# leggedrobotics/qed-splatter

Hardware: AMD Instinct MI355X
Metric: train iters/sec @ 1080p, 500k Gaussians (fwd + loss + bwd + Adam; camera-steps/s over all GPUs) (higher is better)
Workload: dtype f32

## Files before the change

### qed_splatter_amd/_lib.py

```python
from __future__ import annotations

import ctypes as C
import os
import types
from pathlib import Path

_LIB = None
LIB_PATH = Path(__file__).resolve().parent / "lib" / "libqed_splat.so"

_P = C.c_void_p
_I = C.c_int32
_L = C.c_int64
_F = C.c_float
_U = C.c_uint32
_D = C.c_double
_Q = C.c_uint64
SIGNATURES = {
    "qed_version": (C.c_int, []),
    "qed_last_error": (C.c_char_p, []),
    "qed_camera_setup": (C.c_int, [_I, _P, _P, _P, _P, _P]),
    "qed_project_fwd": (C.c_int, [_I, _I, _P, _P, _P, _P, _P, _I, _P, _I, _I, _P, _P, _I, _I, _I, _I, _F, _F, _F,
                                  _F, _U, _P, _P, _P, _P, _P, _P, _P, _P, _P, _P, _P, _P, _P, _P]),
    "qed_project_bwd": (C.c_int, [_I, _I, _P, _P, _P, _P, _P, _I, _P, _I, _I, _P, _P, _I, _I, _F, _U, _P, _P, _P,
                                  _P, _P, _P, _P, _I, _P, _I, _P, _P, _P]),
# ... 121 lines not shown
F_LOG_SCALES = 2
F_LOGIT_OPAC = 4
F_DEPTH_CHANNEL = 8
F_SIGMOID_COLORS = 16
F_TIGHT_TILES = 32
F_CAMERA_C2W = 128
F_SH_GRAD_COMPACT = 64
SPLAT_FLOATS = 12
VSPLAT_FLOATS = 16
SH_JAC_FLOATS = 10
STATUS_WORDS = 4
TILE = 16
CL_TILE_WAVES, CL_QUADRANT_WAVES, CL_HALF_AND_HALF, CL_NO_CULL, CL_ORDER_READY = 1, 2, 3, 4, 8
NN_NATURAL_ORDER, NN_AUTO_CELL = 1, 2
KNN_SKIP_FIRST = 4
BIN_AUTO, BIN_TWO_STAGE, BIN_TILE_SORT, BIN_BUCKET = 0, 1, 2, 3


def bin_mode() -> int:
    return {"two": BIN_TWO_STAGE, "til": BIN_TILE_SORT, "buc": BIN_BUCKET}.get(os.environ.get("QED_BIN_MODE", "")[:3],
                                                                            BIN_AUTO)


def composite_launch_flags() -> int:
    f = {"t": CL_TILE_WAVES, "q": CL_QUADRANT_WAVES, "h": CL_HALF_AND_HALF}.get(
        os.environ.get("QED_COMPOSITE_WAVES", "")[:1], 0)
    if os.environ.get("QED_COMPOSITE_NOCULL", "")[:1] == "1":
        f |= CL_NO_CULL
    return f


class QedSplatError(RuntimeError):
    pass


ABI_VERSION = 4


def load():
    global _LIB
    if _LIB is not None:
        return _LIB
    import torch
    path = Path(os.environ.get("QED_SPLAT_LIB", LIB_PATH))
    if not path.exists():
        raise QedSplatError(
# ... 102 lines not shown
```

### qed_splatter_amd/binning.py

```python
from __future__ import annotations

import time
import warnings
import weakref
from typing import Dict

import torch

from . import _lib as L


def pinned_slot():
    import ctypes
    host = torch.zeros(4, dtype=torch.int32).pin_memory()
    dptr = ctypes.c_void_p()
    L.check(L.load().qed_host_device_pointer(host.data_ptr(), ctypes.addressof(dptr)), "qed_host_device_pointer")
    return host.numpy(), dptr.value, host


class _Workspace:

    HEADROOM = 2.0
    POLL_TIMEOUT_S = 20.0

# ... 126 lines not shown
                  size=None, tile_masks=None, capture_slot=None):
    lib = L.load()
    dev = means2d.device
    ws = _workspace(dev)
    n_tiles = tile_w * tile_h
    key = (tuple(size) if size is not None else (tile_w, tile_h), N, C)
    n_isect = ws.n_isect
    offsets = torch.empty(C * n_tiles + 1, dtype=torch.int32, device=dev)
    capturing = torch.cuda.is_current_stream_capturing()
    if capturing:
        if not ws.may_capture(key):
            raise L.QedSplatError("run one eager call of this shape (image size, number of Gaussians, cameras) before "
                                  "capturing: it calibrates the intersection capacity")
        sync = False
    else:
        ws.poll_pending()
        if not ws.may_skip_readback(key):
            sync = True
    if ws.capacity == 0:
        ws.capacity = max(1 << 16, 8 * C * N)
    mode = L.bin_mode()
    if mode == L.BIN_AUTO and ws.m_seen.get(key, 0) > 0:
        mode = L.BIN_BUCKET if int(1.25 * ws.m_seen[key]) <= 1024 * C * n_tiles else L.BIN_TWO_STAGE
    host = host_ptr = None
    if not sync and not capturing:
        host, host_ptr = ws.host_slot()
    elif capturing and capture_slot is not None:
        host, host_ptr = capture_slot
    for _attempt in range(2):
        cap = ws.capacity
        flatten_ids = torch.empty(cap, dtype=torch.int32, device=dev)
        isect_ids = torch.empty(cap, dtype=torch.int64, device=dev) if sync else None
        scratch = torch.empty(int(lib.qed_bin_workspace_bytes(C * N, cap)), dtype=torch.uint8, device=dev)
        L.check(lib.qed_bin_tiles(N, C, L.ptr(means2d), L.ptr(radii), L.ptr(depths), L.ptr(tiles_per_gauss), L.ptr(splats),
                                  L.ptr(tile_masks), L.ptr(block_sums), tile_w, tile_h, cap, mode, L.ptr(flatten_ids), L.ptr(offsets),
                                  L.ptr(n_isect), L.ptr(isect_ids), L.ptr(scratch), scratch.numel(), L.ptr(ws.status),
                                  host_ptr, L.current_stream()), "qed_bin_tiles")
        if capturing:
            return None, flatten_ids, offsets, None
        if not sync:
            ws.arm_pending(host, key)
            return None, flatten_ids, offsets, None
        M, overflow, watchdog = ws.read_words()
        if watchdog:
            ws.watchdog_fired("the radix-sort look-back watchdog fired: the list of this frame is mis-sorted")
        if overflow == 0:
# ... 7 lines not shown
```

### qed_splatter_amd/csrc/isect.hip

```cpp
#include "qed_common.h"

namespace qed {

constexpr int kScanPer = 32;
__global__ void __launch_bounds__(1024)
isect_scan_kernel(const int* __restrict__ block_sums, int n_blocks, int* __restrict__ block_offsets,
                  int* __restrict__ n_isect, long long capacity, int* __restrict__ status) {
    __shared__ long long wave_tot[16];
    __shared__ long long carry_s;
    const int tid = threadIdx.x, lane = tid & 63, wid = tid >> 6;
    if (tid == 0) carry_s = 0;
    __syncthreads();
    for (int base = 0; base < n_blocks; base += 1024 * kScanPer) {
        const int i0 = base + tid * kScanPer;
        int v[kScanPer];
        const bool vec = (((uintptr_t)block_sums | (uintptr_t)block_offsets) & 15) == 0;
        if (vec && i0 + kScanPer <= n_blocks) {
#pragma unroll
            for (int j = 0; j < kScanPer / 4; ++j) {
                const int4 q = reinterpret_cast<const int4*>(block_sums + i0)[j];
                v[4 * j] = q.x; v[4 * j + 1] = q.y; v[4 * j + 2] = q.z; v[4 * j + 3] = q.w;
            }
        } else {
#pragma unroll
// ... 256 lines not shown
    int v = 0;
    if (i < n_slots) {
        if (order == nullptr) {
            v = tiles_per_gauss[i];
        } else if (slot_bits >= 32) {
            v = tiles_per_gauss[order[i]];
        } else {
            const unsigned o = (unsigned)order[i], marker = (1u << (32 - slot_bits)) - 1u;
            const unsigned c = o >> slot_bits;
            v = c == marker ? tiles_per_gauss[o & ((1u << slot_bits) - 1u)] : (int)c;
        }
    }
    __shared__ int wsum[4];
    v = wave_sum_i(v);
    if ((threadIdx.x & 63) == 0) wsum[threadIdx.x >> 6] = v;
    __syncthreads();
    if (threadIdx.x == 0) block_sums[blockIdx.x] = wsum[0] + wsum[1] + wsum[2] + wsum[3];
}


constexpr int kTileSortKpt = 8;
constexpr int kTileSortItems = 256 * kTileSortKpt;

__device__ __forceinline__ int wave_digit_rank(bool valid, unsigned d, int* cnt, int lane) {
    unsigned long long peers = __ballot(valid);
#pragma unroll
    for (int b = 0; b < 8; ++b) {
        const bool bit = (d >> b) & 1u;
        const unsigned long long bal = __ballot(bit);
        peers &= bit ? bal : ~bal;
    }
    int r = 0;
    if (valid) {
        r = cnt[d] + __popcll(peers & ((1ull << lane) - 1ull));
        if ((peers >> lane) == 1ull) cnt[d] = r + 1;
    }
    return r;
}


constexpr int kTileWaveKpt = 8;
constexpr int kTileWaveItems = 64 * kTileWaveKpt;
constexpr int kTileBuckets = 512;
constexpr int kTileBucketMax = 12;

__device__ __forceinline__ void wave_lds_fence() {
    __builtin_amdgcn_fence(__ATOMIC_ACQ_REL, "wavefront");
    __builtin_amdgcn_wave_barrier();
}

__device__ __forceinline__ void tile_sort_wave(int start, int n, int lane, uint2* __restrict__ kv, int* __restrict__ cnt,
                                               const int* __restrict__ vals_in, const float* __restrict__ depths,
                                               int* __restrict__ vals_out) {
    if (n == 1) {
        if (lane == 0) vals_out[start] = vals_in[start];
        return;
    }
    const int rows = (n + 63) >> 6;
    unsigned key[kTileWaveKpt];
    int val[kTileWaveKpt], rank[kTileWaveKpt];
#pragma unroll
    for (int k = 0; k < kTileWaveKpt; ++k) {
        if (k >= rows) break;
        const int li = k * 64 + lane;
        val[k] = vals_in[start + (li < n ? li : n - 1)];
    }
    unsigned kmin = 0xFFFFFFFFu, kmax = 0u;
#pragma unroll
    for (int k = 0; k < kTileWaveKpt; ++k) {
        if (k >= rows) break;
        key[k] = __float_as_uint(depths[val[k]]);
        kmin = min(kmin, key[k]);
        kmax = max(kmax, key[k]);
    }
#pragma unroll
    for (int o = 32; o > 0; o >>= 1) {
        kmin = min(kmin, (unsigned)__shfl_xor((int)kmin, o, 64));
        kmax = max(kmax, (unsigned)__shfl_xor((int)kmax, o, 64));
    }
    if (kmin == kmax) {
#pragma unroll
        for (int k = 0; k < kTileWaveKpt; ++k) {
            if (k >= rows) break;
            if (k * 64 + lane < n) vals_out[start + k * 64 + lane] = val[k];
        }
        return;
    }
    const float scale = 511.99f / (float)(kmax - kmin);
    unsigned bkt[kTileWaveKpt];
    *reinterpret_cast<int4*>(&cnt[8 * lane]) = make_int4(0, 0, 0, 0);
    *reinterpret_cast<int4*>(&cnt[8 * lane + 4]) = make_int4(0, 0, 0, 0);
    wave_lds_fence();
#pragma unroll
    for (int k = 0; k < kTileWaveKpt; ++k) {
        if (k >= rows) break;
        bkt[k] = min((unsigned)((float)(key[k] - kmin) * scale), (unsigned)(kTileBuckets - 1));
        rank[k] = k * 64 + lane < n ? atomicAdd(&cnt[bkt[k]], 1) : 0;
    }
    wave_lds_fence();
    int largest;
    {
        const int4 c0 = *reinterpret_cast<const int4*>(&cnt[8 * lane]);
        const int4 c1 = *reinterpret_cast<const int4*>(&cnt[8 * lane + 4]);
        largest = max(max(max(c0.x, c0.y), max(c0.z, c0.w)), max(max(c1.x, c1.y), max(c1.z, c1.w)));
        const int tot = c0.x + c0.y + c0.z + c0.w + c1.x + c1.y + c1.z + c1.w;
        int x = tot;
#pragma unroll
        for (int o = 1; o < 64; o <<= 1) {
            const int y = __shfl_up(x, o, 64);
            if (lane >= o) x += y;
        }
#pragma unroll
        for (int o = 32; o > 0; o >>= 1) largest = max(largest, __shfl_xor(largest, o, 64));
        int b = x - tot;
        int4 e0, e1;
        e0.x = b; b += c0.x; e0.y = b; b += c0.y; e0.z = b; b += c0.z; e0.w = b; b += c0.w;
        e1.x = b; b += c1.x; e1.y = b; b += c1.y; e1.z = b; b += c1.z; e1.w = b;
        *reinterpret_cast<int4*>(&cnt[8 * lane]) = e0;
        *reinterpret_cast<int4*>(&cnt[8 * lane + 4]) = e1;
    }
    wave_lds_fence();
    if (largest <= kTileBucketMax) {
#pragma unroll
        for (int k = 0; k < kTileWaveKpt; ++k) {
            if (k >= rows) break;
            if (k * 64 + lane < n) kv[cnt[bkt[k]] + rank[k]] = make_uint2(key[k], (unsigned)val[k]);
        }
        wave_lds_fence();
#pragma unroll
        for (int k = 0; k < kTileWaveKpt; ++k) {
            if (k >= rows) break;
            const int li = k * 64 + lane;
            if (li < n) {
                const int b0 = cnt[bkt[k]];
                const int b1 = bkt[k] + 1 < kTileBuckets ? cnt[bkt[k] + 1] : n;
                int before = 0;
                for (int j = b0; j < b1; ++j) {
                    const unsigned other = kv[j].x;
                    before += (other < key[k]) | ((other == key[k]) & ((int)kv[j].y < val[k]));
                }
                vals_out[start + b0 + before] = val[k];
            }
        }
        return;
    }
    unsigned* skeys = reinterpret_cast<unsigned*>(kv);
    int* svals = reinterpret_cast<int*>(kv) + kTileWaveItems;
    for (int pass = 0; pass < 4; ++pass) {
        const int shift = 8 * pass;
        *reinterpret_cast<int4*>(&cnt[4 * lane]) = make_int4(0, 0, 0, 0);
        wave_lds_fence();
#pragma unroll
        for (int k = 0; k < kTileWaveKpt; ++k) {
            if (k >= rows) break;
            rank[k] = wave_digit_rank(k * 64 + lane < n, (key[k] >> shift) & 255u, cnt, lane);
        }
        wave_lds_fence();
        const int4 c = *reinterpret_cast<const int4*>(&cnt[4 * lane]);
// ... 16 lines not shown
            const int li = k * 64 + lane;
            if (li < n) {
                const int pos = skip ? li : cnt[(key[k] >> shift) & 255u] + rank[k];
                if (last) vals_out[start + pos] = val[k];
                else { skeys[pos] = key[k]; svals[pos] = val[k]; }
            }
        }
        if (last) break;
        wave_lds_fence();
#pragma unroll
        for (int k = 0; k < kTileWaveKpt; ++k) {
            if (k >= rows) break;
            const int li = k * 64 + lane;
            if (li < n) { key[k] = skeys[li]; val[k] = svals[li]; }
        }
        wave_lds_fence();
    }
}

__device__ __forceinline__ void tile_sort_long_run(int start, int n, const int* __restrict__ vals_in,
                                                   const float* __restrict__ depths, int* __restrict__ vals_out,
                                                   unsigned* __restrict__ gk0, unsigned* __restrict__ gk1,
                                                   int* __restrict__ gv0, int* __restrict__ gv1, unsigned* s_keys,
                                                   int* s_vals, int (*s_cnt)[256], int* s_base, int* s_wsum, int* s_skip) {
    const int tid = threadIdx.x, lane = tid & 63, wid = tid >> 6;
    auto digit_scan = [&](int tot) {
        int x = tot;
#pragma unroll
        for (int o = 1; o < 64; o <<= 1) {
            const int y = __shfl_up(x, o, 64);
            if (lane >= o) x += y;
        }
        if (lane == 63) s_wsum[wid] = x;
        __syncthreads();
        int wb = 0;
        for (int w = 0; w < wid; ++w) wb += s_wsum[w];
        return wb + x - tot;
    };
    if (n <= kTileSortItems) {
        unsigned key[kTileSortKpt];
        int val[kTileSortKpt], rank[kTileSortKpt];
        const int Q = ((n + 255) >> 8) << 6;
        const int rows = Q >> 6;
        const int wbase = wid * Q;
        auto mine = [&](int k) { return wbase + 64 * k + lane < n; };
        if (tid < 4) s_skip[tid] = 0;
#pragma unroll
// ... 3 lines not shown
            val[k] = vals_in[start + (li < n ? li : n - 1)];
        }
#pragma unroll
        for (int k = 0; k < kTileSortKpt; ++k) {
            if (k >= rows) break;
            key[k] = __float_as_uint(depths[val[k]]);
        }
        for (int pass = 0; pass < 4; ++pass) {
            const int shift = 8 * pass;
#pragma unroll
            for (int w = 0; w < 4; ++w) s_cnt[w][tid] = 0;
            __syncthreads();
#pragma unroll
            for (int k = 0; k < kTileSortKpt; ++k) {
                if (k >= rows) break;
                rank[k] = wave_digit_rank(mine(k), (key[k] >> shift) & 255u, s_cnt[wid], lane);
            }
            __syncthreads();
            {
                int c[4], tot = 0;
#pragma unroll
                for (int w = 0; w < 4; ++w) c[w] = s_cnt[w][tid];
#pragma unroll
                for (int w = 0; w < 4; ++w) { s_cnt[w][tid] = tot; tot += c[w]; }
                if (tot == n) s_skip[pass] = 1;
                s_base[tid] = digit_scan(tot);
            }
            __syncthreads();
            const bool skip = s_skip[pass] != 0;
            const bool last = pass == 3;
            if (skip && !last) continue;
#pragma unroll
            for (int k = 0; k < kTileSortKpt; ++k) {
                if (k >= rows) break;
                if (mine(k)) {
                    const unsigned d = (key[k] >> shift) & 255u;
                    const int pos = skip ? wbase + k * 64 + lane : s_base[d] + s_cnt[wid][d] + rank[k];
                    if (last) vals_out[start + pos] = val[k];
                    else { s_keys[pos] = key[k]; s_vals[pos] = val[k]; }
                }
            }
            if (last) break;
            __syncthreads();
#pragma unroll
            for (int k = 0; k < kTileSortKpt; ++k) {
                if (k >= rows) break;
                if (mine(k)) { key[k] = s_keys[wbase + k * 64 + lane]; val[k] = s_vals[wbase + k * 64 + lane]; }
// ... 10 lines not shown
        s_base[tid] = 0;
        __syncthreads();
        for (int i = tid; i < n; i += 256) {
            const unsigned kk = ksrc ? ksrc[start + i] : __float_as_uint(depths[vsrc[start + i]]);
            atomicAdd(&s_base[(kk >> shift) & 255u], 1);
        }
        __syncthreads();
        const int tot = s_base[tid];
        const int base = digit_scan(tot);
        __syncthreads();
        s_base[tid] = base;
        __syncthreads();
        for (int row = 0; row < n; row += 256) {
            const int i = row + tid;
            const bool valid = i < n;
            const int vv = valid ? vsrc[start + i] : 0;
            const unsigned kk = valid ? (ksrc ? ksrc[start + i] : __float_as_uint(depths[vv])) : 0u;
            const unsigned d = (kk >> shift) & 255u;
#pragma unroll
            for (int w = 0; w < 4; ++w) s_cnt[w][tid] = 0;
            __syncthreads();
            const int r = wave_digit_rank(valid, d, s_cnt[wid], lane);
            __syncthreads();
            {
                int c[4], t2 = 0;
#pragma unroll
                for (int w = 0; w < 4; ++w) c[w] = s_cnt[w][tid];
                const int cur = s_base[tid];
#pragma unroll
                for (int w = 0; w < 4; ++w) { s_cnt[w][tid] = cur + t2; t2 += c[w]; }
                __syncthreads();
                s_base[tid] = cur + t2;
            }
            __syncthreads();
            if (valid) {
                const int pos = s_cnt[wid][d] + r;
                vdst[start + pos] = vv;
                if (pass < 3) kdst[start + pos] = kk;
            }
            __syncthreads();
        }
        __threadfence_block();
        __syncthreads();
        ksrc = kdst;
        vsrc = vdst;
    }
}

__global__ void __launch_bounds__(256)
tile_depth_sort_kernel(const int* __restrict__ offsets, const int* __restrict__ vals_in, const float* __restrict__ depths,
                       int* __restrict__ vals_out, unsigned* __restrict__ gk0, unsigned* __restrict__ gk1,
                       int* __restrict__ gv0, int* __restrict__ gv1, int n_tiles_total) {
    __shared__ __attribute__((aligned(16))) uint2 s_kv[4][kTileWaveItems];
    __shared__ __attribute__((aligned(16))) int s_cnt[4][kTileBuckets];
    __shared__ int s_wsum[4], s_skip[4];
    const int lane = threadIdx.x & 63, wid = threadIdx.x >> 6;
    const int tile = blockIdx.x * 4 + wid;
    int start = 0, n = 0;
    if (tile < n_tiles_total) { start = offsets[tile]; n = offsets[tile + 1] - start; }
    if (n >= 1 && n <= kTileWaveItems) tile_sort_wave(start, n, lane, s_kv[wid], s_cnt[wid], vals_in, depths, vals_out);
    if (!__syncthreads_or(n > kTileWaveItems)) return;
    static_assert(sizeof(s_kv) >= kTileSortItems * 8 && sizeof(s_cnt) >= (4 * 256 + 256) * 4, "LDS aliasing");
    unsigned* keys = reinterpret_cast<unsigned*>(&s_kv[0][0]);
    int* vals = reinterpret_cast<int*>(keys + kTileSortItems);
    int (*cnt)[256] = reinterpret_cast<int (*)[256]>(&s_cnt[0][0]);
    int* base = &s_cnt[0][0] + 4 * 256;
    for (int j = 0; j < 4; ++j) {
        const int t = blockIdx.x * 4 + j;
        if (t >= n_tiles_total) break;
        const int s0 = offsets[t], m = offsets[t + 1] - s0;
        if (m <= kTileWaveItems) continue;
        __syncthreads();
        tile_sort_long_run(s0, m, vals_in, depths, vals_out, gk0, gk1, gv0, gv1, keys, vals, cnt, base, s_wsum, s_skip);
    }
}

constexpr int kPartThreads = 1024;
constexpr int kPartWaves = kPartThreads / 64;
constexpr int kPartRows = 16;
constexpr int kPartStage = 32768;

__global__ void __launch_bounds__(kPartThreads)
bucket_partition_kernel(const unsigned* __restrict__ keys, const int* __restrict__ vals, const int* __restrict__ n_dev,
                        const int* __restrict__ bucket_tot, int low_bits, int tile_bits, int n_tiles,
                        int n_tiles_total, int* __restrict__ vals_out, unsigned* __restrict__ keys_out,
                        int* __restrict__ offsets, const int* __restrict__ status, int* __restrict__ host_words) {
    __shared__ int s_cnt[kPartWaves][256];
    __shared__ int s_base[256];
    __shared__ int s_wsum[4][2];
    __shared__ int s_stage[kPartStage];
    const int tid = threadIdx.x, lane = tid & 63, wid = tid >> 6;
    const int b = blockIdx.x;
    const int n = n_dev[0];
    if (b == 0 && tid == 0) {
        offsets[n_tiles_total] = n;
        if (host_words != nullptr) {
            *reinterpret_cast<int4*>(host_words) = make_int4(n, status[0], status[1], 0);
            __threadfence_system();
        }
    }
    const unsigned dmask = (1u << low_bits) - 1u;
    int before = 0, size = 0;
    if (tid < 256) {
        const int t = bucket_tot[tid];
        before = tid < b ? t : 0;
        if (tid == b) size = t;
    }
    before = wave_sum_i(before); size = wave_sum_i(size);
    if (wid < 4 && lane == 0) { s_wsum[wid][0] = before; s_wsum[wid][1] = size; }
    for (int i = tid; i < kPartWaves * 256; i += kPartThreads) (&s_cnt[0][0])[i] = 0;
    __syncthreads();
    const int start = s_wsum[0][0] + s_wsum[1][0] + s_wsum[2][0] + s_wsum[3][0];
    const int m = s_wsum[0][1] + s_wsum[1][1] + s_wsum[2][1] + s_wsum[3][1];
    const int rpw = ((m + 63) / 64 + kPartWaves - 1) / kPartWaves;
    const int seg0 = min(wid * rpw * 64, m), seg1 = min(seg0 + rpw * 64, m);
    const unsigned* kin = keys + start;
    const int* vin = vals + start;
    unsigned k0[kPartRows];
    int v0[kPartRows];
#pragma unroll
    for (int j = 0; j < kPartRows; ++j) {
        const int i = seg0 + 64 * j + lane;
        const int ic = i < seg1 ? i : max(seg1 - 1, 0);
        k0[j] = seg1 > seg0 ? kin[ic] : 0u;
        v0[j] = seg1 > seg0 ? vin[ic] : 0;
    }
#pragma unroll
    for (int j = 0; j < kPartRows; ++j)
        if (seg0 + 64 * j + lane < seg1) atomicAdd(&s_cnt[wid][k0[j] & dmask], 1);
    for (int r0 = seg0 + 64 * kPartRows; r0 < seg1; r0 += 64 * kPartRows) {
        unsigned k[kPartRows];
#pragma unroll
        for (int j = 0; j < kPartRows; ++j) {
            const int i = r0 + 64 * j + lane;
            k[j] = kin[i < seg1 ? i : seg1 - 1];
        }
#pragma unroll
        for (int j = 0; j < kPartRows; ++j)
            if (r0 + 64 * j + lane < seg1) atomicAdd(&s_cnt[wid][k[j] & dmask], 1);
    }
    __syncthreads();
    int tot = 0, x = 0;
    if (tid < 256) {
#pragma unroll
        for (int w = 0; w < kPartWaves; ++w) { const int c = s_cnt[w][tid]; s_cnt[w][tid] = tot; tot += c; }
        x = tot;
#pragma unroll
        for (int o = 1; o < 64; o <<= 1) {
            const int y = __shfl_up(x, o, 64);
            if (lane >= o) x += y;
        }
        if (lane == 63) s_wsum[wid][0] = x;
    }
    __syncthreads();
    if (tid < 256) {
        int wb = 0;
        for (int w = 0; w < wid; ++w) wb += s_wsum[w][0];
        const int base = wb + x - tot;
        s_base[tid] = base;
        if (tid <= (int)dmask) {
            const unsigned key = ((unsigned)b << low_bits) | (unsigned)tid;
            const unsigned t = key & ((1u << tile_bits) - 1u);
            const long long lin = (long long)(key >> tile_bits) * n_tiles + t;
            if ((int)t < n_tiles && lin < n_tiles_total) offsets[lin] = start + base;
        }
    }
    __syncthreads();
    const bool staged = m <= kPartStage;
    const unsigned long long lt = (1ull << lane) - 1ull;
    auto place = [&](int r0, const unsigned (&k)[kPartRows], const int (&v)[kPartRows]) {
#pragma unroll
        for (int j = 0; j < kPartRows; ++j) {
            if (r0 + 64 * j >= seg1) break;
            const bool valid = r0 + 64 * j + lane < seg1;
            const unsigned d = k[j] & dmask;
            unsigned long long peers = __ballot(valid);
            for (int bit = 0; bit < low_bits; ++bit) {
                const bool on = (d >> bit) & 1u;
                const unsigned long long bal = __ballot(on);
                peers &= on ? bal : ~bal;
            }
            if (valid) {
                const int r = s_cnt[wid][d] + __popcll(peers & lt);
                if ((peers >> lane) == 1ull) s_cnt[wid][d] = r + 1;
                const int pos = s_base[d] + r;
                if (staged) s_stage[pos] = v[j];
                else vals_out[start + pos] = v[j];
                if (keys_out != nullptr) keys_out[start + pos] = k[j];
            }
        }
    };
    place(seg0, k0, v0);
    for (int r0 = seg0 + 64 * kPartRows; r0 < seg1; r0 += 64 * kPartRows) {
        unsigned k[kPartRows];
        int v[kPartRows];
#pragma unroll
        for (int j = 0; j < kPartRows; ++j) {
            const int i = r0 + 64 * j + lane;
            const int ic = i < seg1 ? i : seg1 - 1;
            k[j] = kin[ic];
            v[j] = vin[ic];
        }
        place(r0, k, v);
    }
    if (!staged) return;
    __syncthreads();
    for (int i = tid; i < m; i += kPartThreads) vals_out[start + i] = s_stage[i];
}

__global__ void __launch_bounds__(256)
isect_ids_kernel(const unsigned* __restrict__ tile_keys, const int* __restrict__ flatten_ids,
                 const float* __restrict__ depths, const int* __restrict__ n_dev, unsigned long long* __restrict__ out) {
    const int i = blockIdx.x * 256 + threadIdx.x;
    if (i < n_dev[0])
        out[i] = ((unsigned long long)tile_keys[i] << 32) | (unsigned long long)__float_as_uint(depths[flatten_ids[i]]);
}

}

using namespace qed;

static long long align256(long long x) { return (x + 255) & ~255ll; }

// ... 17 lines not shown
    L.keysA0 = o; o += align256(4 * S);
    L.keysA1 = o; o += align256(4 * S);
    L.valsA0 = o; o += align256(4 * S);
    L.valsA1 = o; o += align256(4 * S);
    L.block_sums = o; o += align256(4 * nblk);
    L.block_offsets = o; o += align256(4 * nblk);
    L.keysB0 = o; o += align256(4 * cap);
    L.keysB1 = o; o += align256(4 * cap);
    L.valsB = o; o += align256(4 * cap);
    L.sort_ws_bytes = sort32_workspace_bytes(S > cap ? S : cap);
    L.sort_ws = o; o += align256(L.sort_ws_bytes);
    L.tk1 = o; o += align256(4 * cap);
    L.tv0 = o; o += align256(4 * cap);
    L.tv1 = o; o += align256(4 * cap);
    L.total = o;
    return L;
}

extern "C" int64_t qed_bin_workspace_bytes(int64_t n_slots, int64_t capacity) {
    if (n_slots < 0 || capacity < 0) return QED_E_INVALID_ARG;
    return bin_layout(n_slots, capacity).total;
}

extern "C" int qed_bin_tiles(int32_t N, int32_t C, const float* means2d, const int32_t* radii, const float* depths,
                             const int32_t* tiles_per_gauss, const float* splats, const uint64_t* tile_masks,
                             const int32_t* block_sums_in, int32_t tile_w, int32_t tile_h, int64_t capacity,
                             int32_t mode, int32_t* flatten_ids,
                             int32_t* offsets, int32_t* n_isect, uint64_t* isect_ids, void* workspace,
                             int64_t workspace_bytes, int32_t* status, int32_t* host_words, void* stream) {
    QED_REQUIRE(N >= 0 && C >= 1 && tile_w > 0 && tile_h > 0, "bad extents");
    QED_REQUIRE(splats == nullptr || (tile_w <= 1023 && tile_h <= 2047), "packed tile rectangles need tile_w <= 1023");
    QED_REQUIRE(tile_masks == nullptr || splats != nullptr, "tile_masks index the rectangles of the splat records");
    QED_REQUIRE(((uintptr_t)tile_masks & 15) == 0, "tile_masks must be 16-byte aligned");
    QED_REQUIRE(capacity >= 0 && capacity < (1ll << 30), "capacity out of range");
    QED_REQUIRE(offsets && n_isect && status && workspace, "null buffers");
    QED_REQUIRE(((uintptr_t)host_words & 15) == 0, "host_words must be 16-byte aligned");
    const long long S = (long long)C * N;
    QED_REQUIRE(S < (1ll << 30), "too many (camera, Gaussian) slots");
    const long long n_tot = (long long)C * tile_w * tile_h;
    int tile_bits = 1;
    while ((1ll << tile_bits) <= (long long)tile_w * tile_h) ++tile_bits;
    int cam_bits = 0;
    while ((1 << cam_bits) < C) ++cam_bits;
    QED_REQUIRE(tile_bits + cam_bits <= 32, "camera/tile key does not fit 32 bits");
    const BinLayout L = bin_layout(S, capacity);
    if (workspace_bytes < L.total) {
        set_error("qed_bin_tiles: workspace too small (%lld < %lld)", (long long)workspace_bytes, L.total);
        return QED_E_WORKSPACE;
    }
    hipStream_t st = (hipStream_t)stream;
    char* w = (char*)workspace;
    int* n_slots_dev = (int*)(w + L.n_slots_dev);
    unsigned* kA0 = (unsigned*)(w + L.keysA0); unsigned* kA1 = (unsigned*)(w + L.keysA1);
// ... 20 lines not shown
                               depths, tiles_per_gauss, bsums, tile_w, tile_h, tile_bits, n_isect, order, kB0, vals_out,
                               splats, (long long)capacity, status, (const unsigned long long*)tile_masks, slot_mask);
        } else {
            hipLaunchKernelGGL(isect_scan_kernel, dim3(1), dim3(1024), 0, st, bsums, (int)gridS, block_offsets, n_isect,
                               (long long)capacity, status);
            hipLaunchKernelGGL((isect_emit_kernel<unsigned, false>), dim3(gridS), dim3(256), 0, st, N, C, means2d, radii,
                               depths, tiles_per_gauss, (const int*)block_offsets, tile_w, tile_h, tile_bits, n_isect, order,
                               kB0, vals_out, splats, (long long)capacity, status, (const unsigned long long*)tile_masks,
                               slot_mask);
        }
    };
    if (mode == QED_BIN_AUTO) mode = capacity <= 1024 * n_tot ? QED_BIN_BUCKET : QED_BIN_TWO_STAGE;
    if (mode == QED_BIN_BUCKET && tile_bits + cam_bits > 16) mode = QED_BIN_TILE_SORT;
    if (mode == QED_BIN_BUCKET) {
        const int* bsums = block_sums_in;
        if (bsums == nullptr) {
            hipLaunchKernelGGL(count_sorted_kernel, dim3(gridS), dim3(256), 0, st, (int)S, (const int*)nullptr,
                               tiles_per_gauss, block_sums);
            bsums = block_sums;
        }
        launch_emit(bsums, (const int*)nullptr, flatten_ids);
        const int end_bit = tile_bits + cam_bits;
        const int low_bits = end_bit > 8 ? end_bit - 8 : 0;
        const int* bucket_tot = nullptr;
        int rc = sort_pass_u32(kB0, flatten_ids, kB1, vB, n_isect, capacity, low_bits, end_bit - low_bits, sort_ws,
                               L.sort_ws_bytes, &bucket_tot, st);
        if (rc != QED_OK) return rc;
        const long long max_key = ((long long)(C - 1) << tile_bits) | (long long)(tile_w * tile_h - 1);
        const unsigned n_buckets = (unsigned)((max_key >> low_bits) + 1);
        int* v_tiles = (int*)(w + L.tv0);
        unsigned* k_tiles = isect_ids != nullptr ? (unsigned*)(w + L.tk1) : nullptr;
        hipLaunchKernelGGL(bucket_partition_kernel, dim3(n_buckets), dim3(kPartThreads), 0, st, (const unsigned*)kB1,
                           (const int*)vB, (const int*)n_isect, bucket_tot, low_bits, tile_bits, tile_w * tile_h,
                           (int)n_tot, v_tiles, k_tiles, offsets, (const int*)status, host_words);
        hipLaunchKernelGGL(tile_depth_sort_kernel, dim3((unsigned)((n_tot + 3) / 4)), dim3(256), 0, st,
                           (const int*)offsets, (const int*)v_tiles, depths, flatten_ids, kB0, kB1, vB,
                           (int*)(w + L.tv1), (int)n_tot);
        if (isect_ids != nullptr)
            hipLaunchKernelGGL(isect_ids_kernel, dim3((unsigned)((capacity + 255) / 256)), dim3(256), 0, st,
                               (const unsigned*)k_tiles, (const int*)flatten_ids, depths, (const int*)n_isect,
                               (unsigned long long*)isect_ids);
        return check_launch("qed_bin_tiles");
    }
    if (mode == QED_BIN_TILE_SORT) {
        const int* bsums = block_sums_in;
        if (bsums == nullptr) {
            hipLaunchKernelGGL(count_sorted_kernel, dim3(gridS), dim3(256), 0, st, (int)S, (const int*)nullptr,
                               tiles_per_gauss, block_sums);
            bsums = block_sums;
        }
        const int end_bit = tile_bits + cam_bits;
        const int passes = (end_bit + 7) / 8;
        int* v_first = (passes & 1) ? flatten_ids : vB;
        int* v_alt = (passes & 1) ? vB : flatten_ids;
        launch_emit(bsums, (const int*)nullptr, v_first);
        const int which = sort_pairs_u32(kB0, v_first, kB1, v_alt, n_isect, capacity, end_bit, sort_ws, L.sort_ws_bytes,
                                         status, st);
// ... 83 lines not shown
```

### qed_splatter_amd/csrc/radix_sort.hip

```cpp
#include "qed_common.h"

namespace qed {

constexpr int kSortThreads = 256;
constexpr int kSortWaves = kSortThreads / 64;
constexpr int kRadixBits = 8;
constexpr int kRadix = 1 << kRadixBits;

template <typename KeyT, int KPT>
struct SortCfg {
    static constexpr int kItems = kSortThreads * KPT;
};

template <typename KeyT>
__device__ __forceinline__ unsigned digit_of(KeyT k, int shift, unsigned mask) {
    return (unsigned)(k >> shift) & mask;
}

template <typename KeyT, int KPT>
__global__ void __launch_bounds__(kSortThreads)
sort_hist_kernel(const KeyT* __restrict__ keys, const int* __restrict__ n_dev, int shift, unsigned mask,
                 int nblocks_max, int* __restrict__ hist) {
    constexpr int kItems = SortCfg<KeyT, KPT>::kItems;
    const int n = n_dev[0];
// ... 49 lines not shown
            int x = v;
#pragma unroll
            for (int o = 1; o < 64; o <<= 1) {
                const int y = __shfl_up(x, o, 64);
                if (lane >= o) x += y;
            }
            if (lane == 63) s_wave[wid] = x;
            __syncthreads();
            int wb = 0;
            for (int w = 0; w < wid; ++w) wb += s_wave[w];
            const int carry = s_carry;
            if (i < nb) row[i] = carry + wb + x - v;
            __syncthreads();
            if (tid == kSortThreads - 1) s_carry = carry + wb + x;
            __syncthreads();
        }
    }
    if (tid == 0) digit_tot[blockIdx.x] = s_carry;
}

constexpr unsigned kLbPartial = 1u << 30, kLbInclusive = 2u << 30, kLbValue = (1u << 30) - 1u;
constexpr int kLbSpinLimit = 1 << 18;

template <typename KeyT, int KPT, bool LOOKBACK>
__global__ void __launch_bounds__(kSortThreads)
sort_scatter_kernel(const KeyT* __restrict__ keys_in, const int* __restrict__ vals_in, KeyT* __restrict__ keys_out,
                    int* __restrict__ vals_out, const int* __restrict__ n_dev, int shift, unsigned mask,
                    int nblocks_max, const int* __restrict__ hist, const int* __restrict__ digit_tot,
                    unsigned* __restrict__ lookback, int* __restrict__ ticket, int* __restrict__ status) {
    constexpr int kItems = SortCfg<KeyT, KPT>::kItems;
    const int n = n_dev[0];
    int tile = blockIdx.x;
    if constexpr (LOOKBACK) {
        __shared__ int s_tile;
        if (threadIdx.x == 0) s_tile = atomicAdd(ticket, 1);
        __syncthreads();
        tile = s_tile;
    }
    const long long base = (long long)tile * kItems;
    if (base >= n) return;
    const int block_n = (int)min((long long)kItems, (long long)n - base);

    __shared__ KeyT s_keys[kItems];
    __shared__ int s_vals[kItems];
    __shared__ int s_cnt[kSortWaves][kRadix];
    __shared__ int s_lbase[kRadix];
    __shared__ int s_gofs[kRadix];
// ... 93 lines not shown
        s_lbase[tid] = lbase;
        s_gofs[tid] = gbase - lbase;
    }
    __syncthreads();

#pragma unroll
    for (int k = 0; k < KPT; ++k) {
        const int li = wbase + k * 64 + lane;
        if (li < block_n) {
            const unsigned d = digit_of<KeyT>(key[k], shift, mask);
            const int pos = s_lbase[d] + s_cnt[wid][d] + rank[k];
            s_keys[pos] = key[k];
            s_vals[pos] = val[k];
        }
    }
    __syncthreads();
#pragma unroll
    for (int k = 0; k < KPT; ++k) {
        const int pos = k * kSortThreads + tid;
        if (pos < block_n) {
            const KeyT kk = s_keys[pos];
            const unsigned d = digit_of<KeyT>(kk, shift, mask);
            const long long dst = (long long)s_gofs[d] + pos;
            keys_out[dst] = kk;
            vals_out[dst] = s_vals[pos];
        }
    }
}

template <typename KeyT, int PASSES>
__global__ void __launch_bounds__(kSortThreads)
sort_global_hist_kernel(const KeyT* __restrict__ keys, const int* __restrict__ n_dev, int end_bit,
                        int* __restrict__ ghist) {
    __shared__ int s_h[PASSES][kRadix];
    const int n = n_dev[0];
#pragma unroll
    for (int p = 0; p < PASSES; ++p) s_h[p][threadIdx.x] = 0;
    __syncthreads();
    for (long long i = (long long)blockIdx.x * kSortThreads + threadIdx.x; i < n; i += (long long)gridDim.x * kSortThreads) {
        const KeyT k = keys[i];
#pragma unroll
        for (int p = 0; p < PASSES; ++p) {
            const int shift = p * kRadixBits;
            if (shift < end_bit) {
                const int bits = min(kRadixBits, end_bit - shift);
                atomicAdd(&s_h[p][digit_of<KeyT>(k, shift, (1u << bits) - 1u)], 1);
            }
        }
// ... 104 lines not shown
                                                     workspace_bytes, status, st);
    return sort_pairs_impl<unsigned, kKpt32>(keys, vals, keys_alt, vals_alt, n_dev, capacity, end_bit, workspace,
                                             workspace_bytes, status, st);
}

template <int KPT>
static int sort_pass_impl(const unsigned* kin, const int* vin, unsigned* kout, int* vout, const int* n_dev,
                          long long capacity, int shift, int bits, void* workspace, long long workspace_bytes,
                          const int** digit_tot_out, hipStream_t st) {
    constexpr int kItems = SortCfg<unsigned, KPT>::kItems;
    const int nblocks_max = (int)((capacity + kItems - 1) / kItems);
    const long long need = sort_workspace_need<unsigned, KPT>(capacity);
    if (nblocks_max == 0 || workspace_bytes < need) {
        set_error("sort_pass_u32: empty capacity or workspace too small (%lld < %lld)", workspace_bytes, need);
        return QED_E_WORKSPACE;
    }
    int* hist = (int*)workspace;
    int* digit_tot = hist + (long long)kRadix * nblocks_max;
    const unsigned mask = (1u << bits) - 1u;
    hipLaunchKernelGGL((sort_hist_kernel<unsigned, KPT>), dim3(nblocks_max), dim3(kSortThreads), 0, st, kin, n_dev,
                       shift, mask, nblocks_max, hist);
    hipLaunchKernelGGL((sort_scan_kernel<kItems>), dim3(kRadix), dim3(kSortThreads), 0, st, n_dev, nblocks_max, hist,
                       digit_tot);
    hipLaunchKernelGGL((sort_scatter_kernel<unsigned, KPT, false>), dim3(nblocks_max), dim3(kSortThreads), 0, st, kin,
                       vin, kout, vout, n_dev, shift, mask, nblocks_max, (const int*)hist, (const int*)digit_tot,
                       (unsigned*)nullptr, (int*)nullptr, (int*)nullptr);
    *digit_tot_out = digit_tot;
    return check_launch("sort_pass_u32");
}

int sort_pass_u32(const unsigned* kin, const int* vin, unsigned* kout, int* vout, const int* n_dev, long long capacity,
                  int shift, int bits, void* workspace, long long workspace_bytes, const int** digit_tot,
                  hipStream_t st) {
    if (bits < 1 || bits > kRadixBits) { set_error("sort_pass_u32: 1..8 digit bits"); return QED_E_INVALID_ARG; }
    if (capacity >= kSortLongList)
        return sort_pass_impl<kKpt32Long>(kin, vin, kout, vout, n_dev, capacity, shift, bits, workspace,
                                          workspace_bytes, digit_tot, st);
    return sort_pass_impl<kKpt32>(kin, vin, kout, vout, n_dev, capacity, shift, bits, workspace, workspace_bytes,
                                  digit_tot, st);
}

}

using namespace qed;

extern "C" int64_t qed_sort_workspace_bytes(int64_t capacity) {
    if (capacity < 0) return QED_E_INVALID_ARG;
    return sort_workspace_need<unsigned long long, kKpt64>(capacity);
}
// ... 14 lines not shown
```

Measured before the change: 1171.

## Pack low key bits into value word in bucket sort; shrink tile-sort LDS counters to 16-bit

The first radix pass now folds the low key bits into the upper bits of the value word when the slot count fits, so it writes no separate key array and the bucket partition reads only values. The tile depth sort uses 16-bit packed bucket counters in LDS, drops a barrier in the per-tile radix pass, and checks tile lengths from global offsets instead of a block-wide OR. It also requests eight waves per EU to raise occupancy. This cuts global memory traffic in binning and LDS footprint, at the cost of extra bit manipulation and a limit on how many slots the packed form can address.

```diff
diff --git a/qed_splatter_amd/_lib.py b/qed_splatter_amd/_lib.py
--- a/qed_splatter_amd/_lib.py
+++ b/qed_splatter_amd/_lib.py
@@ -167,6 +167,19 @@
                                                                             BIN_AUTO)
 
 
+BIN_PAIR_FORM = 0x100
+
+
+def bin_flags() -> int:
+    return BIN_PAIR_FORM if os.environ.get("QED_BIN_WORD", "")[:4] == "pair" else 0
+
+
+def bin_word_fits(n_slots: int, low_bits: int) -> bool:
+    fn = load()._cdll.qed_bin_word_fits
+    fn.restype, fn.argtypes = C.c_int32, (C.c_int64, C.c_int32)
+    return bool(fn(n_slots, low_bits))
+
+
 def composite_launch_flags() -> int:
     f = {"t": CL_TILE_WAVES, "q": CL_QUADRANT_WAVES, "h": CL_HALF_AND_HALF}.get(
         os.environ.get("QED_COMPOSITE_WAVES", "")[:1], 0)
diff --git a/qed_splatter_amd/binning.py b/qed_splatter_amd/binning.py
--- a/qed_splatter_amd/binning.py
+++ b/qed_splatter_amd/binning.py
@@ -172,6 +172,7 @@
     mode = L.bin_mode()
     if mode == L.BIN_AUTO and ws.m_seen.get(key, 0) > 0:
         mode = L.BIN_BUCKET if int(1.25 * ws.m_seen[key]) <= 1024 * C * n_tiles else L.BIN_TWO_STAGE
+    mode |= L.bin_flags()
     host = host_ptr = None
     if not sync and not capturing:
         host, host_ptr = ws.host_slot()
diff --git a/qed_splatter_amd/csrc/isect.hip b/qed_splatter_amd/csrc/isect.hip
--- a/qed_splatter_amd/csrc/isect.hip
+++ b/qed_splatter_amd/csrc/isect.hip
@@ -302,7 +302,8 @@
 constexpr int kTileSortKpt = 8;
 constexpr int kTileSortItems = 256 * kTileSortKpt;
 
-__device__ __forceinline__ int wave_digit_rank(bool valid, unsigned d, int* cnt, int lane) {
+template <typename CntT>
+__device__ __forceinline__ int wave_digit_rank(bool valid, unsigned d, CntT* cnt, int lane) {
     unsigned long long peers = __ballot(valid);
 #pragma unroll
     for (int b = 0; b < 8; ++b) {
@@ -312,8 +313,8 @@
     }
     int r = 0;
     if (valid) {
-        r = cnt[d] + __popcll(peers & ((1ull << lane) - 1ull));
-        if ((peers >> lane) == 1ull) cnt[d] = r + 1;
+        r = (int)cnt[d] + __popcll(peers & ((1ull << lane) - 1ull));
+        if ((peers >> lane) == 1ull) cnt[d] = (CntT)(r + 1);
     }
     return r;
 }
@@ -332,6 +333,7 @@
 __device__ __forceinline__ void tile_sort_wave(int start, int n, int lane, uint2* __restrict__ kv, int* __restrict__ cnt,
                                                const int* __restrict__ vals_in, const float* __restrict__ depths,
                                                int* __restrict__ vals_out) {
+    const unsigned short* cnt16 = reinterpret_cast<const unsigned short*>(cnt);
     if (n == 1) {
         if (lane == 0) vals_out[start] = vals_in[start];
         return;
@@ -368,22 +370,23 @@
     }
     const float scale = 511.99f / (float)(kmax - kmin);
     unsigned bkt[kTileWaveKpt];
-    *reinterpret_cast<int4*>(&cnt[8 * lane]) = make_int4(0, 0, 0, 0);
-    *reinterpret_cast<int4*>(&cnt[8 * lane + 4]) = make_int4(0, 0, 0, 0);
+    *reinterpret_cast<int4*>(&cnt[4 * lane]) = make_int4(0, 0, 0, 0);
     wave_lds_fence();
 #pragma unroll
     for (int k = 0; k < kTileWaveKpt; ++k) {
         if (k >= rows) break;
         bkt[k] = min((unsigned)((float)(key[k] - kmin) * scale), (unsigned)(kTileBuckets - 1));
-        rank[k] = k * 64 + lane < n ? atomicAdd(&cnt[bkt[k]], 1) : 0;
+        const int half = 16 * (int)(bkt[k] & 1u);
+        rank[k] = k * 64 + lane < n ? (atomicAdd(&cnt[bkt[k] >> 1], 1 << half) >> half) & 0xFFFF : 0;
     }
     wave_lds_fence();
     int largest;
     {
-        const int4 c0 = *reinterpret_cast<const int4*>(&cnt[8 * lane]);
-        const int4 c1 = *reinterpret_cast<const int4*>(&cnt[8 * lane + 4]);
-        largest = max(max(max(c0.x, c0.y), max(c0.z, c0.w)), max(max(c1.x, c1.y), max(c1.z, c1.w)));
-        const int tot = c0.x + c0.y + c0.z + c0.w + c1.x + c1.y + c1.z + c1.w;
+        const int4 c = *reinterpret_cast<const int4*>(&cnt[4 * lane]);
+        const int c0 = c.x & 0xFFFF, c1 = (unsigned)c.x >> 16, c2 = c.y & 0xFFFF, c3 = (unsigned)c.y >> 16;
+        const int c4 = c.z & 0xFFFF, c5 = (unsigned)c.z >> 16, c6 = c.w & 0xFFFF, c7 = (unsigned)c.w >> 16;
+        largest = max(max(max(c0, c1), max(c2, c3)), max(max(c4, c5), max(c6, c7)));
+        const int tot = c0 + c1 + c2 + c3 + c4 + c5 + c6 + c7;
         int x = tot;
 #pragma unroll
         for (int o = 1; o < 64; o <<= 1) {
@@ -392,19 +395,16 @@
         }
 #pragma unroll
         for (int o = 32; o > 0; o >>= 1) largest = max(largest, __shfl_xor(largest, o, 64));
-        int b = x - tot;
-        int4 e0, e1;
-        e0.x = b; b += c0.x; e0.y = b; b += c0.y; e0.z = b; b += c0.z; e0.w = b; b += c0.w;
-        e1.x = b; b += c1.x; e1.y = b; b += c1.y; e1.z = b; b += c1.z; e1.w = b;
-        *reinterpret_cast<int4*>(&cnt[8 * lane]) = e0;
-        *reinterpret_cast<int4*>(&cnt[8 * lane + 4]) = e1;
+        const int b0 = x - tot, b1 = b0 + c0, b2 = b1 + c1, b3 = b2 + c2, b4 = b3 + c3, b5 = b4 + c4, b6 = b5 + c5,
+                  b7 = b6 + c6;
+        *reinterpret_cast<int4*>(&cnt[4 * lane]) = make_int4(b0 | (b1 << 16), b2 | (b3 << 16), b4 | (b5 << 16), b6 | (b7 << 16));
     }
     wave_lds_fence();
     if (largest <= kTileBucketMax) {
 #pragma unroll
         for (int k = 0; k < kTileWaveKpt; ++k) {
             if (k >= rows) break;
-            if (k * 64 + lane < n) kv[cnt[bkt[k]] + rank[k]] = make_uint2(key[k], (unsigned)val[k]);
+            if (k * 64 + lane < n) kv[cnt16[bkt[k]] + rank[k]] = make_uint2(key[k], (unsigned)val[k]);
         }
         wave_lds_fence();
 #pragma unroll
@@ -412,8 +412,8 @@
             if (k >= rows) break;
             const int li = k * 64 + lane;
             if (li < n) {
-                const int b0 = cnt[bkt[k]];
-                const int b1 = bkt[k] + 1 < kTileBuckets ? cnt[bkt[k] + 1] : n;
+                const int b0 = cnt16[bkt[k]];
+                const int b1 = bkt[k] + 1 < kTileBuckets ? cnt16[bkt[k] + 1] : n;
                 int before = 0;
                 for (int j = b0; j < b1; ++j) {
                     const unsigned other = kv[j].x;
@@ -476,7 +476,8 @@
                                                    const float* __restrict__ depths, int* __restrict__ vals_out,
                                                    unsigned* __restrict__ gk0, unsigned* __restrict__ gk1,
                                                    int* __restrict__ gv0, int* __restrict__ gv1, unsigned* s_keys,
-                                                   int* s_vals, int (*s_cnt)[256], int* s_base, int* s_wsum, int* s_skip) {
+                                                   int* s_vals, unsigned short (*s_cnt)[256], int* s_base, int* s_wsum,
+                                                   int* s_skip) {
     const int tid = threadIdx.x, lane = tid & 63, wid = tid >> 6;
     auto digit_scan = [&](int tot) {
         int x = tot;
@@ -526,7 +527,7 @@
 #pragma unroll
                 for (int w = 0; w < 4; ++w) c[w] = s_cnt[w][tid];
 #pragma unroll
-                for (int w = 0; w < 4; ++w) { s_cnt[w][tid] = tot; tot += c[w]; }
+                for (int w = 0; w < 4; ++w) { s_cnt[w][tid] = (unsigned short)tot; tot += c[w]; }
                 if (tot == n) s_skip[pass] = 1;
                 s_base[tid] = digit_scan(tot);
             }
@@ -583,23 +584,22 @@
             __syncthreads();
             const int r = wave_digit_rank(valid, d, s_cnt[wid], lane);
             __syncthreads();
+            int t2 = 0;
             {
-                int c[4], t2 = 0;
+                int c[4];
 #pragma unroll
                 for (int w = 0; w < 4; ++w) c[w] = s_cnt[w][tid];
-                const int cur = s_base[tid];
-#pragma unroll
-                for (int w = 0; w < 4; ++w) { s_cnt[w][tid] = cur + t2; t2 += c[w]; }
-                __syncthreads();
-                s_base[tid] = cur + t2;
+#pragma unroll
+                for (int w = 0; w < 4; ++w) { s_cnt[w][tid] = (unsigned short)t2; t2 += c[w]; }
             }
             __syncthreads();
             if (valid) {
-                const int pos = s_cnt[wid][d] + r;
+                const int pos = s_base[d] + s_cnt[wid][d] + r;
                 vdst[start + pos] = vv;
                 if (pass < 3) kdst[start + pos] = kk;
             }
             __syncthreads();
+            s_base[tid] += t2;
         }
         __threadfence_block();
         __syncthreads();
@@ -608,24 +608,32 @@
     }
 }
 
-__global__ void __launch_bounds__(256)
+__global__ void __launch_bounds__(256) __attribute__((amdgpu_waves_per_eu(8, 8)))
 tile_depth_sort_kernel(const int* __restrict__ offsets, const int* __restrict__ vals_in, const float* __restrict__ depths,
                        int* __restrict__ vals_out, unsigned* __restrict__ gk0, unsigned* __restrict__ gk1,
                        int* __restrict__ gv0, int* __restrict__ gv1, int n_tiles_total) {
     __shared__ __attribute__((aligned(16))) uint2 s_kv[4][kTileWaveItems];
-    __shared__ __attribute__((aligned(16))) int s_cnt[4][kTileBuckets];
-    __shared__ int s_wsum[4], s_skip[4];
+    __shared__ __attribute__((aligned(16))) int s_cnt[4][kTileBuckets / 2];
     const int lane = threadIdx.x & 63, wid = threadIdx.x >> 6;
     const int tile = blockIdx.x * 4 + wid;
     int start = 0, n = 0;
     if (tile < n_tiles_total) { start = offsets[tile]; n = offsets[tile + 1] - start; }
     if (n >= 1 && n <= kTileWaveItems) tile_sort_wave(start, n, lane, s_kv[wid], s_cnt[wid], vals_in, depths, vals_out);
-    if (!__syncthreads_or(n > kTileWaveItems)) return;
-    static_assert(sizeof(s_kv) >= kTileSortItems * 8 && sizeof(s_cnt) >= (4 * 256 + 256) * 4, "LDS aliasing");
+    bool any_long = false;
+#pragma unroll
+    for (int j = 0; j < 4; ++j) {
+        const int t = min((int)blockIdx.x * 4 + j, n_tiles_total - 1);
+        any_long |= offsets[t + 1] - offsets[t] > kTileWaveItems;
+    }
+    if (!any_long) return;
+    static_assert(sizeof(s_kv) >= kTileSortItems * 8 && sizeof(s_cnt) >= 4 * 256 * 2 + 256 * 4 + 8 * 4, "LDS aliasing");
+    static_assert(sizeof(s_kv) + sizeof(s_cnt) <= 20480, "eight workgroups per CU");
     unsigned* keys = reinterpret_cast<unsigned*>(&s_kv[0][0]);
     int* vals = reinterpret_cast<int*>(keys + kTileSortItems);
-    int (*cnt)[256] = reinterpret_cast<int (*)[256]>(&s_cnt[0][0]);
-    int* base = &s_cnt[0][0] + 4 * 256;
+    unsigned short (*cnt)[256] = reinterpret_cast<unsigned short (*)[256]>(&s_cnt[0][0]);
+    int* base = &s_cnt[0][0] + 4 * 256 / 2;
+    int* s_wsum = base + 256;
+    int* s_skip = s_wsum + 4;
     for (int j = 0; j < 4; ++j) {
         const int t = blockIdx.x * 4 + j;
         if (t >= n_tiles_total) break;
@@ -641,6 +649,7 @@
 constexpr int kPartRows = 16;
 constexpr int kPartStage = 32768;
 
+template <bool PACKED>
 __global__ void __launch_bounds__(kPartThreads)
 bucket_partition_kernel(const unsigned* __restrict__ keys, const int* __restrict__ vals, const int* __restrict__ n_dev,
                         const int* __restrict__ bucket_tot, int low_bits, int tile_bits, int n_tiles,
@@ -661,6 +670,10 @@
         }
     }
     const unsigned dmask = (1u << low_bits) - 1u;
+    const int wshift = 32 - low_bits;
+    const unsigned vmask = low_bits > 0 ? (1u << wshift) - 1u : 0xFFFFFFFFu;
+    auto digit = [&](unsigned k, int v) { return PACKED ? (low_bits > 0 ? (unsigned)v >> wshift : 0u) : k & dmask; };
+    auto value = [&](int v) { return PACKED ? (int)((unsigned)v & vmask) : v; };
     int before = 0, size = 0;
     if (tid < 256) {
         const int t = bucket_tot[tid];
@@ -675,7 +688,7 @@
     const int m = s_wsum[0][1] + s_wsum[1][1] + s_wsum[2][1] + s_wsum[3][1];
     const int rpw = ((m + 63) / 64 + kPartWaves - 1) / kPartWaves;
     const int seg0 = min(wid * rpw * 64, m), seg1 = min(seg0 + rpw * 64, m);
-    const unsigned* kin = keys + start;
+    const unsigned* kin = PACKED ? nullptr : keys + start;
     const int* vin = vals + start;
     unsigned k0[kPartRows];
     int v0[kPartRows];
@@ -683,22 +696,23 @@
     for (int j = 0; j < kPartRows; ++j) {
         const int i = seg0 + 64 * j + lane;
         const int ic = i < seg1 ? i : max(seg1 - 1, 0);
-        k0[j] = seg1 > seg0 ? kin[ic] : 0u;
+        k0[j] = !PACKED && seg1 > seg0 ? kin[ic] : 0u;
         v0[j] = seg1 > seg0 ? vin[ic] : 0;
     }
 #pragma unroll
     for (int j = 0; j < kPartRows; ++j)
-        if (seg0 + 64 * j + lane < seg1) atomicAdd(&s_cnt[wid][k0[j] & dmask], 1);
+        if (seg0 + 64 * j + lane < seg1) atomicAdd(&s_cnt[wid][digit(k0[j], v0[j])], 1);
     for (int r0 = seg0 + 64 * kPartRows; r0 < seg1; r0 += 64 * kPartRows) {
-        unsigned k[kPartRows];
+        unsigned d[kPartRows];
 #pragma unroll
         for (int j = 0; j < kPartRows; ++j) {
             const int i = r0 + 64 * j + lane;
-            k[j] = kin[i < seg1 ? i : seg1 - 1];
+            const int ic = i < seg1 ? i : seg1 - 1;
+            d[j] = PACKED ? digit(0u, vin[ic]) : digit(kin[ic], 0);
         }
 #pragma unroll
         for (int j = 0; j < kPartRows; ++j)
-            if (r0 + 64 * j + lane < seg1) atomicAdd(&s_cnt[wid][k[j] & dmask], 1);
+            if (r0 + 64 * j + lane < seg1) atomicAdd(&s_cnt[wid][d[j]], 1);
     }
     __syncthreads();
     int tot = 0, x = 0;
@@ -734,7 +748,7 @@
         for (int j = 0; j < kPartRows; ++j) {
             if (r0 + 64 * j >= seg1) break;
             const bool valid = r0 + 64 * j + lane < seg1;
-            const unsigned d = k[j] & dmask;
+            const unsigned d = digit(k[j], v[j]);
             unsigned long long peers = __ballot(valid);
             for (int bit = 0; bit < low_bits; ++bit) {
                 const bool on = (d >> bit) & 1u;
@@ -745,9 +759,9 @@
                 const int r = s_cnt[wid][d] + __popcll(peers & lt);
                 if ((peers >> lane) == 1ull) s_cnt[wid][d] = r + 1;
                 const int pos = s_base[d] + r;
-                if (staged) s_stage[pos] = v[j];
-                else vals_out[start + pos] = v[j];
-                if (keys_out != nullptr) keys_out[start + pos] = k[j];
+                if (staged) s_stage[pos] = value(v[j]);
+                else vals_out[start + pos] = value(v[j]);
+                if (keys_out != nullptr) keys_out[start + pos] = ((unsigned)b << low_bits) | d;
             }
         }
     };
@@ -759,7 +773,7 @@
         for (int j = 0; j < kPartRows; ++j) {
             const int i = r0 + 64 * j + lane;
             const int ic = i < seg1 ? i : seg1 - 1;
-            k[j] = kin[ic];
+            k[j] = PACKED ? 0u : kin[ic];
             v[j] = vin[ic];
         }
         place(r0, k, v);
@@ -823,6 +837,12 @@
     return bin_layout(n_slots, capacity).total;
 }
 
+extern "C" int32_t qed_bin_word_fits(int64_t n_slots, int32_t low_bits) {
+    return low_bits >= 0 && low_bits <= 8 && n_slots >= 0 && n_slots < (1ll << (32 - low_bits)) ? 1 : 0;
+}
+
+constexpr int32_t kBinPairForm = 0x100;
+
 extern "C" int qed_bin_tiles(int32_t N, int32_t C, const float* means2d, const int32_t* radii, const float* depths,
                              const int32_t* tiles_per_gauss, const float* splats, const uint64_t* tile_masks,
                              const int32_t* block_sums_in, int32_t tile_w, int32_t tile_h, int64_t capacity,
@@ -830,6 +850,8 @@
                              int32_t* offsets, int32_t* n_isect, uint64_t* isect_ids, void* workspace,
                              int64_t workspace_bytes, int32_t* status, int32_t* host_words, void* stream) {
     QED_REQUIRE(N >= 0 && C >= 1 && tile_w > 0 && tile_h > 0, "bad extents");
+    const bool pair_form = (mode & kBinPairForm) != 0;
+    mode &= ~kBinPairForm;
     QED_REQUIRE(splats == nullptr || (tile_w <= 1023 && tile_h <= 2047), "packed tile rectangles need tile_w <= 1023");
     QED_REQUIRE(tile_masks == nullptr || splats != nullptr, "tile_masks index the rectangles of the splat records");
     QED_REQUIRE(((uintptr_t)tile_masks & 15) == 0, "tile_masks must be 16-byte aligned");
@@ -896,17 +918,24 @@
         launch_emit(bsums, (const int*)nullptr, flatten_ids);
         const int end_bit = tile_bits + cam_bits;
         const int low_bits = end_bit > 8 ? end_bit - 8 : 0;
+        const bool packed = !pair_form && qed_bin_word_fits(S, low_bits) != 0;
         const int* bucket_tot = nullptr;
-        int rc = sort_pass_u32(kB0, flatten_ids, kB1, vB, n_isect, capacity, low_bits, end_bit - low_bits, sort_ws,
-                               L.sort_ws_bytes, &bucket_tot, st);
+        int rc = sort_pass_u32(kB0, flatten_ids, packed ? nullptr : kB1, vB, n_isect, capacity, low_bits,
+                               end_bit - low_bits, sort_ws, L.sort_ws_bytes, &bucket_tot, st);
         if (rc != QED_OK) return rc;
         const long long max_key = ((long long)(C - 1) << tile_bits) | (long long)(tile_w * tile_h - 1);
         const unsigned n_buckets = (unsigned)((max_key >> low_bits) + 1);
         int* v_tiles = (int*)(w + L.tv0);
         unsigned* k_tiles = isect_ids != nullptr ? (unsigned*)(w + L.tk1) : nullptr;
-        hipLaunchKernelGGL(bucket_partition_kernel, dim3(n_buckets), dim3(kPartThreads), 0, st, (const unsigned*)kB1,
-                           (const int*)vB, (const int*)n_isect, bucket_tot, low_bits, tile_bits, tile_w * tile_h,
-                           (int)n_tot, v_tiles, k_tiles, offsets, (const int*)status, host_words);
+        if (packed)
+            hipLaunchKernelGGL(bucket_partition_kernel<true>, dim3(n_buckets), dim3(kPartThreads), 0, st,
+                               (const unsigned*)nullptr, (const int*)vB, (const int*)n_isect, bucket_tot, low_bits,
+                               tile_bits, tile_w * tile_h, (int)n_tot, v_tiles, k_tiles, offsets, (const int*)status,
+                               host_words);
+        else
+            hipLaunchKernelGGL(bucket_partition_kernel<false>, dim3(n_buckets), dim3(kPartThreads), 0, st,
+                               (const unsigned*)kB1, (const int*)vB, (const int*)n_isect, bucket_tot, low_bits, tile_bits,
+                               tile_w * tile_h, (int)n_tot, v_tiles, k_tiles, offsets, (const int*)status, host_words);
         hipLaunchKernelGGL(tile_depth_sort_kernel, dim3((unsigned)((n_tot + 3) / 4)), dim3(256), 0, st,
                            (const int*)offsets, (const int*)v_tiles, depths, flatten_ids, kB0, kB1, vB,
                            (int*)(w + L.tv1), (int)n_tot);
diff --git a/qed_splatter_amd/csrc/radix_sort.hip b/qed_splatter_amd/csrc/radix_sort.hip
--- a/qed_splatter_amd/csrc/radix_sort.hip
+++ b/qed_splatter_amd/csrc/radix_sort.hip
@@ -95,7 +95,7 @@
 constexpr unsigned kLbPartial = 1u << 30, kLbInclusive = 2u << 30, kLbValue = (1u << 30) - 1u;
 constexpr int kLbSpinLimit = 1 << 18;
 
-template <typename KeyT, int KPT, bool LOOKBACK>
+template <typename KeyT, int KPT, bool LOOKBACK, bool PACK = false>
 __global__ void __launch_bounds__(kSortThreads)
 sort_scatter_kernel(const KeyT* __restrict__ keys_in, const int* __restrict__ vals_in, KeyT* __restrict__ keys_out,
                     int* __restrict__ vals_out, const int* __restrict__ n_dev, int shift, unsigned mask,
@@ -235,8 +235,13 @@
             const KeyT kk = s_keys[pos];
             const unsigned d = digit_of<KeyT>(kk, shift, mask);
             const long long dst = (long long)s_gofs[d] + pos;
-            keys_out[dst] = kk;
-            vals_out[dst] = s_vals[pos];
+            if constexpr (PACK) {
+                const unsigned low = (unsigned)kk & ((1u << shift) - 1u);
+                vals_out[dst] = shift > 0 ? (int)((low << (32 - shift)) | (unsigned)s_vals[pos]) : s_vals[pos];
+            } else {
+                keys_out[dst] = kk;
+                vals_out[dst] = s_vals[pos];
+            }
         }
     }
 }
@@ -387,9 +392,14 @@
                        shift, mask, nblocks_max, hist);
     hipLaunchKernelGGL((sort_scan_kernel<kItems>), dim3(kRadix), dim3(kSortThreads), 0, st, n_dev, nblocks_max, hist,
                        digit_tot);
-    hipLaunchKernelGGL((sort_scatter_kernel<unsigned, KPT, false>), dim3(nblocks_max), dim3(kSortThreads), 0, st, kin,
-                       vin, kout, vout, n_dev, shift, mask, nblocks_max, (const int*)hist, (const int*)digit_tot,
-                       (unsigned*)nullptr, (int*)nullptr, (int*)nullptr);
+    if (kout == nullptr)
+        hipLaunchKernelGGL((sort_scatter_kernel<unsigned, KPT, false, true>), dim3(nblocks_max), dim3(kSortThreads), 0, st,
+                           kin, vin, kout, vout, n_dev, shift, mask, nblocks_max, (const int*)hist, (const int*)digit_tot,
+                           (unsigned*)nullptr, (int*)nullptr, (int*)nullptr);
+    else
+        hipLaunchKernelGGL((sort_scatter_kernel<unsigned, KPT, false>), dim3(nblocks_max), dim3(kSortThreads), 0, st, kin,
+                           vin, kout, vout, n_dev, shift, mask, nblocks_max, (const int*)hist, (const int*)digit_tot,
+                           (unsigned*)nullptr, (int*)nullptr, (int*)nullptr);
     *digit_tot_out = digit_tot;
     return check_launch("sort_pass_u32");
 }
```

Result: no change. 1179 (median of 5 runs) (+0.7%).
